# Andreas-Edling/raytracer-rs

Hardware: AMD Instinct MI355X
Metric: Mrays/s (whole node) + ms/frame, 1920x1080x64spp thai2.dae (higher is better)
Workload: dtype f32

## Files before the change

include/mi355rt.h:

```cpp
#ifndef MI355RT_H
#define MI355RT_H

#include <stddef.h>
#include <stdint.h>

#ifdef __cplusplus
extern "C" {
#endif

#define MI355RT_OK            0
#define MI355RT_E_INVALID    -1
#define MI355RT_E_NO_DEVICE  -2
#define MI355RT_E_LOAD       -3
#define MI355RT_E_HIP        -4

#define MI355RT_DEFAULT_TRIANGLES_PER_LEAF 70u
#define MI355RT_DEFAULT_STRIPE_ROWS 4u

#define MI355RT_FLAG_FIX_ROW_INDEX  1u
#define MI355RT_FLAG_COUNT_STEPS    2u
#define MI355RT_FLAG_TIME_KERNELS   4u
#define MI355RT_FLAG_OCTREE_SEMANTICS 8u
#define MI355RT_FLAG_TRUE_CLOSEST_HIT 32u
#define MI355RT_FLAG_GROUP_SHARES_DEVICE 16u
// ... 200 lines not shown
void mi355rt_lens_default(mi355rt_lens* lens);
int  mi355rt_set_lens(mi355rt_handle* h, const mi355rt_lens* lens);
int  mi355rt_get_lens(const mi355rt_handle* h, mi355rt_lens* lens);
int  mi355rt_lens_ray(const float rot16[16], const float orient16[16], const float max_xy[2], uint32_t width, uint32_t height, uint32_t flags,
                      const mi355rt_lens* lens, uint32_t pixel, float xi1, float xi2, float l1, float l2, float ray6[6]);
int  mi355rt_lens_rays(mi355rt_handle* h, uint32_t spp, uint32_t where, float* rays6, size_t nrays);

int mi355rt_get_sample_table(const mi355rt_handle* h, float* out);
int mi355rt_debug_sample(mi355rt_handle* h, uint32_t pixel, uint32_t sampleno, float color3[3], float* node_L, size_t nodes);
int mi355rt_debug_numerics(mi355rt_handle* h, const float* a, const float* b, size_t n, float* quot, float* root, float* pow32);
int mi355rt_debug_slab(mi355rt_handle* h, const float* inv_rays6, const float* cubes6, size_t n, uint8_t* hit, float* tmin);
uint32_t mi355rt_tree_nodes(const mi355rt_handle* h);
int mi355rt_debug_speculation(const mi355rt_handle* h, uint64_t out[2]);
int mi355rt_debug_light_map(const float* tri_verts, uint32_t ntri, const float light[3], double pad, uint32_t res, float* out_dist2, double* nearest);
int mi355rt_debug_reflect_mask(const float* tri_verts, uint32_t ntri, double pad, uint32_t bins, uint64_t work_budget, uint32_t* out_words, double info[8]);

int mi355rt_debug_wide_bvh(const float* tri_verts, uint32_t ntri, uint32_t out[8]);

int mi355rt_accel_stats(const mi355rt_handle* h, uint32_t out[8]);
int mi355rt_reflect_mask_info(const mi355rt_handle* h, double out[4]);
int mi355rt_debug_rays_read(const mi355rt_handle* h, uint64_t* out);
int mi355rt_bvh_build_info(const mi355rt_handle* h, uint32_t out[2]);
int mi355rt_octree_stats(const mi355rt_handle* h, uint32_t out[8]);
uint32_t mi355rt_device_count(const mi355rt_handle* h);
int mi355rt_debug_gather_rate(mi355rt_handle* h, uint32_t table_nodes, uint32_t steps, double out[3]);
int64_t mi355rt_debug_check_guards(mi355rt_handle* h);
uint64_t mi355rt_hbm_allocated_bytes(const mi355rt_handle* h);
int mi355rt_synchronize(mi355rt_handle* h);

#define MI355RT_COMM_ID_BYTES 128
int mi355rt_comm_unique_id(uint8_t* id128);
int mi355rt_comm_available(mi355rt_handle* h);
int mi355rt_comm_init(mi355rt_handle* h, const uint8_t* id128);
int mi355rt_comm_gather_frame(mi355rt_handle* h, uint32_t root, uint32_t* host_out, size_t n);
int mi355rt_comm_destroy(mi355rt_handle* h);
// ... 12 lines not shown
```

raytracer-rs_amd/__init__.py:

```python
import ctypes as C
import os
import sys
import time
import weakref

import numpy as np

DEFAULT_TRIANGLES_PER_LEAF = 70

FLAG_FIX_ROW_INDEX = 1
FLAG_COUNT_STEPS = 2
FLAG_TIME_KERNELS = 4
FLAG_OCTREE_SEMANTICS = 8
FLAG_GROUP_SHARES_DEVICE = 16
FLAG_TRUE_CLOSEST_HIT = 32
FLAG_DEVICE_LBVH = 64
FLAG_DIRECT_FILM = 128

_HERE = os.path.dirname(os.path.abspath(__file__))
LIB_PATH = os.environ.get("MI355RT_LIB") or os.path.join(_HERE, "libmi355rt.so")
_lib = None


class Material(C.Structure):
# ... 170 lines not shown
    ("mi355rt_trace_rays", C.c_int, [_H, C.c_void_p, C.c_void_p, C.c_size_t, C.c_uint32, C.POINTER(RayOutputs)]),
    ("mi355rt_render_rays", C.c_int, [_H, C.c_void_p, C.c_size_t, C.c_uint32, C.c_uint32, C.POINTER(RayCounts)]),
    ("mi355rt_lens_default", None, [C.POINTER(Lens)]),
    ("mi355rt_set_lens", C.c_int, [_H, C.POINTER(Lens)]),
    ("mi355rt_get_lens", C.c_int, [_H, C.POINTER(Lens)]),
    ("mi355rt_lens_ray", C.c_int, [_F, _F, _F, C.c_uint32, C.c_uint32, C.c_uint32, C.POINTER(Lens), C.c_uint32, C.c_float, C.c_float, C.c_float, C.c_float, _F]),
    ("mi355rt_lens_rays", C.c_int, [_H, C.c_uint32, C.c_uint32, C.c_void_p, C.c_size_t]),
    ("mi355rt_get_sample_table", C.c_int, [_H, _F]),
    ("mi355rt_debug_sample", C.c_int, [_H, C.c_uint32, C.c_uint32, _F, _F, C.c_size_t]),
    ("mi355rt_debug_numerics", C.c_int, [_H, _F, _F, C.c_size_t, _F, _F, _F]),
    ("mi355rt_debug_slab", C.c_int, [_H, _F, _F, C.c_size_t, C.POINTER(C.c_uint8), _F]),
    ("mi355rt_tree_nodes", C.c_uint32, [_H]),
    ("mi355rt_debug_speculation", C.c_int, [_H, C.POINTER(C.c_uint64)]),
    ("mi355rt_debug_light_map", C.c_int, [_F, C.c_uint32, _F, C.c_double, C.c_uint32, _F, C.POINTER(C.c_double)]),
    ("mi355rt_debug_reflect_mask", C.c_int, [_F, C.c_uint32, C.c_double, C.c_uint32, C.c_uint64, _U, C.POINTER(C.c_double)]),
    ("mi355rt_reflect_mask_info", C.c_int, [_H, C.POINTER(C.c_double)]),
    ("mi355rt_debug_rays_read", C.c_int, [_H, C.POINTER(C.c_uint64)]),
    ("mi355rt_debug_wide_bvh", C.c_int, [_F, C.c_uint32, _U]),
    ("mi355rt_accel_stats", C.c_int, [_H, _U]),
    ("mi355rt_octree_stats", C.c_int, [_H, _U]),
    ("mi355rt_bvh_build_info", C.c_int, [_H, _U]),
    ("mi355rt_device_count", C.c_uint32, [_H]),
    ("mi355rt_synchronize", C.c_int, [_H]),
    ("mi355rt_comm_unique_id", C.c_int, [C.POINTER(C.c_uint8)]),
    ("mi355rt_comm_available", C.c_int, [_H]),
    ("mi355rt_comm_init", C.c_int, [_H, C.POINTER(C.c_uint8)]),
    ("mi355rt_comm_gather_frame", C.c_int, [_H, C.c_uint32, _U, C.c_size_t]),
    ("mi355rt_comm_destroy", C.c_int, [_H]),
    ("mi355rt_comm_ranks", C.c_uint32, [_H]),
    ("mi355rt_hbm_allocated_bytes", C.c_uint64, [_H]),
# ... 474 lines not shown

    def debug_slab(self, inv_rays6, cubes6):
        r = np.ascontiguousarray(inv_rays6, np.float32).reshape(-1, 6); c = np.ascontiguousarray(cubes6, np.float32).reshape(-1, 6)
        assert r.shape == c.shape
        hit = np.zeros(r.shape[0], np.uint8); tmin = np.zeros(r.shape[0], np.float32)
        self._check(lib().mi355rt_debug_slab(self._h, _fp(r), _fp(c), r.shape[0], hit.ctypes.data_as(C.POINTER(C.c_uint8)), _fp(tmin)))
        return hit.astype(bool), tmin

    def accel_stats(self):
        out = np.zeros(8, np.uint32)
        self._check(lib().mi355rt_accel_stats(self._h, _up(out)))
        return dict(nodes=int(out[0]), leaves=int(out[1]), max_depth=int(out[2]), max_leaf=int(out[3]),
                    node_bytes=int(out[4]), tri_bytes=int(out[5]), bvh_build_ms=int(out[6]) / 1000.0, octree_build_ms=int(out[7]) / 1000.0)

    def reflect_mask_info(self):
        out = (C.c_double * 4)()
        self._check(lib().mi355rt_reflect_mask_info(self._h, out))
        return dict(bins=int(out[0]), build_ms=float(out[1]), clear_share=float(out[2]), bytes=int(out[3]))

    def debug_rays_read(self):
        out = C.c_uint64(0)
        self._check(lib().mi355rt_debug_rays_read(self._h, C.byref(out)))
        return int(out.value)

    def bvh_build_info(self):
        out = np.zeros(2, np.uint32)
        self._check(lib().mi355rt_bvh_build_info(self._h, _up(out)))
        return dict(on_device=bool(out[0]), device_ms=int(out[1]) / 1000.0)

    def octree_stats(self):
        out = np.zeros(8, np.uint32)
        self._check(lib().mi355rt_octree_stats(self._h, _up(out)))
        return dict(nodes=int(out[0]), inner=int(out[1]), leaves=int(out[2]), empty=int(out[3]), depth=int(out[4]), tri_refs=int(out[5]))
# ... 96 lines not shown

def debug_reflect_mask(tri_verts, pad, bins=8, work_budget=0, min_cos=0.0, pad_angle=0.0):
    v = np.ascontiguousarray(tri_verts, np.float32).reshape(-1, 9)
    info = (C.c_double * 8)()
    info[4], info[5] = float(min_cos), float(pad_angle)
    stride = 6 * bins * bins // 32 + 4
    out = np.zeros((v.shape[0], stride), np.uint32)
    code = lib().mi355rt_debug_reflect_mask(_fp(v), v.shape[0], float(pad), int(bins), int(work_budget), _up(out), info)
    if code != 0:
        raise RuntimeError("mi355rt_debug_reflect_mask failed: %d" % code)
    d = dict(stride=int(info[0]), build_ms=float(info[1]), work=int(info[2]), clear_bits=int(info[3]), min_cos=float(info[4]), pad_angle=float(info[5]),
             bary_margin=float(info[6]), built=bool(info[7]))
    return (out if d["built"] else None), d


def debug_wide_bvh(tri_verts):
    v = np.ascontiguousarray(tri_verts, np.float32).reshape(-1, 9)
    out = (C.c_uint32 * 8)()
    code = lib().mi355rt_debug_wide_bvh(_fp(v), v.shape[0], out)
    if code != 0:
        raise RuntimeError("mi355rt_debug_wide_bvh failed: %d" % code)
    keys = ("wide_nodes", "binary_nodes", "stack_need", "binary_depth", "children", "tris_once_wide", "bad_boxes", "tris_once_binary")
    return dict(zip(keys, (int(x) for x in out)))


def comm_unique_id():
    buf = (C.c_uint8 * 128)()
    if lib().mi355rt_comm_unique_id(buf) != 0:
        raise RuntimeError((lib().mi355rt_last_error(None) or b"").decode() or "mi355rt_comm_unique_id failed")
    return bytes(buf)
# ... 29 lines not shown
```

raytracer-rs_amd/csrc/capi.cpp:

```cpp
#include <cmath>
#include <cstdio>
#include <cstring>
#include <exception>
#include <memory>
#include <string>
#include <vector>
#include "display.hpp"
#include "lightmap.hpp"
#include "reflmask.hpp"
#include "../../include/mi355rt.h"
#include "group.hpp"
#include "lens.hpp"
#include "renderer.hpp"

using namespace mi355rt;

namespace mi355rt { bool comm_unique_id(uint8_t* id128, std::string& err); }

struct mi355rt_handle {
    std::unique_ptr<DeviceGroup> g;
    Renderer* r;
    std::string error;
};

// ... 721 lines not shown
    mi355rt::LightMap lm;
    mi355rt::build_light_map(tri_verts, ntri, light, pad, res, lm);
    std::memcpy(out_dist2, lm.dist2.data(), lm.dist2.size() * sizeof(float));
    if (nearest) *nearest = lm.nearest;
    return MI355RT_OK;
}
int mi355rt_debug_reflect_mask(const float* tri_verts, uint32_t ntri, double pad, uint32_t bins, uint64_t work_budget, uint32_t* out_words, double info[8])
{
    if ((ntri && !tri_verts) || !info || !(pad >= 0.0)) return MI355RT_E_INVALID;
    mi355rt::ReflMask m;
    const double min_cos = info[4] > 0.0 ? info[4] : mi355rt::kReflMinCos, pad_angle = info[5] > 0.0 ? info[5] : mi355rt::kReflPadAngle;
    const bool built = ntri != 0 && mi355rt::build_reflect_mask(tri_verts, ntri, pad, bins, work_budget ? work_budget : ~0ull, m, min_cos, pad_angle);
    info[0] = (double)mi355rt::refl_mask_stride(bins); info[1] = m.build_ms; info[2] = (double)m.work; info[3] = (double)m.clear_bits;
    info[4] = min_cos; info[5] = pad_angle; info[6] = (double)mi355rt::kReflBary; info[7] = built ? 1.0 : 0.0;
    if (built && out_words) std::memcpy(out_words, m.words.data(), m.words.size() * sizeof(uint32_t));
    return MI355RT_OK;
}

namespace {
struct WideWalk {
    const mi355rt::Bvh& b; std::vector<uint32_t> seen; uint32_t children = 0, bad_boxes = 0;
    void below(int32_t ref, double mn[3], double mx[3])
    {
        for (int a = 0; a < 3; ++a) { mn[a] = 1e300; mx[a] = -1e300; }
        if (ref < 0) {
            const uint32_t code = ~(uint32_t)ref, first = code >> 3, cnt = (code & 7u) + 1u;
            for (uint32_t t = first; t < first + cnt && t < b.tris.size(); ++t) {
                const mi355rt::BvhTri& r = b.tris[t];
                if (r.prim < seen.size()) ++seen[r.prim];
                for (int v = 0; v < 3; ++v) for (int a = 0; a < 3; ++a) {
// ... 60 lines not shown
    out[6] = (uint32_t)(h->r->build_ms_[0] * 1000.0); out[7] = (uint32_t)(h->r->build_ms_[1] * 1000.0);
    return MI355RT_OK;
}
int mi355rt_bvh_build_info(const mi355rt_handle* h, uint32_t out[2])
{
    if (!h || !out) return MI355RT_E_INVALID;
    out[0] = h->r->bvh_on_device_ ? 1u : 0u; out[1] = (uint32_t)(h->r->lbvh_device_ms_ * 1000.0);
    return MI355RT_OK;
}
int mi355rt_debug_rays_read(const mi355rt_handle* h, uint64_t* out)
{
    if (!h || !out) return MI355RT_E_INVALID;
    *out = h->r->rays_read_;
    return MI355RT_OK;
}
int mi355rt_reflect_mask_info(const mi355rt_handle* h, double out[4])
{
    if (!h || !out) return MI355RT_E_INVALID;
    std::memcpy(out, h->r->reflect_mask_info_, sizeof h->r->reflect_mask_info_);
    return MI355RT_OK;
}
int mi355rt_octree_stats(const mi355rt_handle* h, uint32_t out[8])
{
    if (!h || !out) return MI355RT_E_INVALID;
    std::memcpy(out, h->r->oct_stats_, sizeof h->r->oct_stats_);
    return MI355RT_OK;
}
uint32_t mi355rt_device_count(const mi355rt_handle* h) { return h ? (uint32_t)h->g->size() : 0u; }

int mi355rt_debug_gather_rate(mi355rt_handle* h, uint32_t table_nodes, uint32_t steps, double out[3])
{
// ... 65 lines not shown
```

raytracer-rs_amd/csrc/device_types.hpp:

```cpp
#pragma once
#include <cstdint>
#include <hip/hip_vector_types.h>

namespace mi355rt {

constexpr uint32_t kNumSamples = 65536;
constexpr uint32_t kSampleMax = 65535;
constexpr uint32_t kMaxRecursions = 3;
constexpr uint32_t kMaxLevels = kMaxRecursions + 1;

constexpr uint32_t kRayRecordBytes = 32;
constexpr uint32_t kShards = 64;
constexpr uint32_t kMaxRounds = kMaxRecursions + 2;
constexpr uint32_t kCullRects = 16;
constexpr uint32_t kMaxCursors = 64;
constexpr uint32_t kCtrlWordsPerRound = kMaxCursors * 16384;
constexpr uint32_t kShadeCursorOffset = 128;
constexpr uint32_t kConfirmCursorOffset = 64;
constexpr uint32_t kLiveCountOffset = 192;

struct DMaterial { float r, g, b; uint32_t kind_tex; };
struct DLight { float px, py, pz, cr, cg, cb;
                float tail2;
                float pad; };
// ... 4 lines not shown
    const void* tris;
    const void* normals;
    const DMaterial* materials;
    const DLight* lights;
    const DTexture* textures;
    const float* texels;
    const void* table;
    const void* oct_nodes;
    const uint32_t* oct_leaf_tris;
    const void* prim_tris;
    const int2* oct_info;
    const uint32_t* tri_home;
    const float* light_maps;
    uint32_t light_map_res;
    const uint32_t* refl_mask;
    uint32_t refl_bins, refl_stride;
    int32_t root;
    uint32_t nlights;
    uint32_t ntri;
    uint32_t oct_single_leaf;
    float oct_root[6];
};

constexpr uint32_t kLensPinhole = 0u, kLensThin = 1u, kLensOrtho = 2u;
struct DLens {
    uint32_t model; float radius, focus, width_world;
    float hw, hh, hw2, hh2;
    float axis[3];
    float mx2, my2;
};
// ... 92 lines not shown
```

raytracer-rs_amd/csrc/kernels.hip:

```cpp
#include <hip/hip_runtime.h>
#include <algorithm>
#include <stdint.h>
#include <stdlib.h>
#include <map>
#include <mutex>
#include <utility>
#include "device_math.hpp"
#include "device_types.hpp"
#include "kernels.hpp"
#include "lens.hpp"
#include "reflmask.hpp"
#include "traverse.hpp"

namespace mi355rt {

typedef const uint32_t __attribute__((address_space(4))) * const_u1_ptr;
constexpr int kBlock = 256;
constexpr int kWavesPerBlock = kBlock / 64;
constexpr uint32_t kMiss = 0xFFFFFFFFu;
constexpr int kPrimaryBlocks = 7;
#ifndef MI355RT_WIDE_BLOCKS
#define MI355RT_WIDE_BLOCKS 5
#endif
constexpr int kConfirmBlocks = 5;
// ... 658 lines not shown
    if (ax >= ay && ax >= az) { m = 0u; vm = vx; va = vy; vb = vz; }
    else if (ay >= az) { m = 1u; vm = vy; va = vx; vb = vz; }
    else { m = 2u; vm = vz; va = vx; vb = vy; }
    const float am = fabsf(vm);
    if (!(am > 0.0f) || !(l2 < 3.0e38f)) return false;
    const float fR = (float)R, u = div_rn(va, am), v = div_rn(vb, am);
    const int i = min(max((int)((u * 0.5f + 0.5f) * fR), 0), (int)R - 1), j = min(max((int)((v * 0.5f + 0.5f) * fR), 0), (int)R - 1);
    const uint32_t face = 2u * m + (vm < 0.0f ? 1u : 0u);
    const float bound = sc.light_maps[((size_t)(li * 6u + face) * R + (uint32_t)i) * R + (uint32_t)j];
    return (l2 * 0.98011f < bound) & (l2 * 1.0002e-4f < lt.tail2);
}

__device__ __forceinline__ uint32_t reflection_record(const DScene& sc, const float4 h)
{
    if (sc.refl_mask == nullptr || !((h.y > kReflBary) & (h.z > kReflBary) & (h.y + h.z < 1.0f - kReflBary))) return kMiss;
    return __float_as_uint(h.w) * sc.refl_stride;
}
__device__ __forceinline__ bool reflection_proves_miss(const DScene& sc, uint32_t rec_first, const f3 n, const f3 bo, const f3 bd)
{
    if (rec_first == kMiss) return false;
    const float ax = fabsf(bd.x), ay = fabsf(bd.y), az = fabsf(bd.z);
    uint32_t m; float vm, va, vb;
    if (ax >= ay && ax >= az) { m = 0u; vm = bd.x; va = bd.y; vb = bd.z; }
    else if (ay >= az) { m = 1u; vm = bd.y; va = bd.x; vb = bd.z; }
    else { m = 2u; vm = bd.z; va = bd.x; vb = bd.y; }
    const float am = fabsf(vm);
    if (!(am > 0.0f)) return false;
    const uint32_t B = sc.refl_bins;
    const float fB = (float)B, u = div_rn(va, am), v = div_rn(vb, am);
    const int i = min(max((int)((u * 0.5f + 0.5f) * fB), 0), (int)B - 1), j = min(max((int)((v * 0.5f + 0.5f) * fB), 0), (int)B - 1);
    const uint32_t bit = ((2u * m + (vm < 0.0f ? 1u : 0u)) * B + (uint32_t)i) * B + (uint32_t)j;
    const uint32_t* __restrict__ rec = sc.refl_mask + rec_first;
    if ((rec[bit >> 5] >> (bit & 31u)) & 1u) return false;
    const float4 g = *(const float4*)(rec + (sc.refl_stride - kReflGuardWords));
    return dot3(sub3(bo, mk3(g.x, g.y, g.z)), n) > g.w;
}

template <bool PRIMARY, class List, bool WALK = false, bool RASTER = false, uint32_t RAYS = kFeedCamera>
__device__ __forceinline__ void shade_chunk(const DScene& sc, const DCamera& cam, const DPass& ps, uint32_t level, uint32_t chunk, const List list,
                                            const float4* __restrict__ in_q, uint32_t in_nrad, uint32_t& out_nrad, uint32_t& out_nshadow,
                                            const float4* __restrict__ hits,
                                            float4* __restrict__ out_q, uint2* __restrict__ out_counts,
                                            float* __restrict__ slot_L, uint32_t* __restrict__ sample_slot,
                                            const uint32_t* __restrict__ film_n, DCounters* counters,
                                            unsigned long long& acc_bounce, unsigned long long& acc_shadow, unsigned long long& acc_hits,
                                            float4* lds_hits = nullptr, unsigned long long* acc_tris = nullptr)
{
    const int lane = lane_id();
    {
        uint32_t n_rad = PRIMARY ? min(ps.chunk, ps.nsamples - chunk * ps.chunk) : in_nrad;
// ... 118 lines not shown
                        pcg4d(a0, a1, a2, a3);
                        uint32_t jx0 = __umulhi(a0, 65535u), jx1 = jx0;
                        if (two) {
                            uint32_t b0 = pixel, b1 = sampleno, b2 = 1u + child1, b3 = ps.seed;
                            pcg4d(b0, b1, b2, b3);
                            jx1 = __umulhi(b0, 65535u);
                        }
                        float4 tv0 = table[jx0], tv1 = table[jx1];
                        hemisphere_walk(table, n, jx0, tv0);
                        if (two) hemisphere_walk(table, n, jx1, tv1);
                        bd0 = mk3(tv0.x, tv0.y, tv0.z); bo0 = add3(hp, sscale(0.00001f, bd0));
                        bd1 = mk3(tv1.x, tv1.y, tv1.z); bo1 = add3(hp, sscale(0.00001f, bd1));
                    }
                    bool make0 = active, make1 = active && two;
                    if (sc.refl_mask != nullptr) {
                        if (make0) make0 = !reflection_proves_miss(sc, refl_rec, n, bo0, bd0);
                        if (make1) make1 = !reflection_proves_miss(sc, refl_rec, n, bo1, bd1);
                        bskipped += (uint32_t)__popcll(__ballot(active && !make0)) + (uint32_t)__popcll(__ballot(active && two && !make1));
                    }
                    uint32_t pos[2] = { 0u, 0u };
                    const uint32_t key0 = make0 ? dir_bin(bd0) : kSortBins, key1 = make1 ? dir_bin(bd1) : kSortBins;
                    for (uint32_t b = 0; b < kSortBins; ++b) {
                        const unsigned long long m0 = __ballot(key0 == b), m1 = __ballot(key1 == b);
                        if (key0 == b) pos[0] = out_front + (uint32_t)__popcll(m0 & lanemask_lt());
                        out_front += (uint32_t)__popcll(m0);
                        if (key1 == b) pos[1] = out_front + (uint32_t)__popcll(m1 & lanemask_lt());
                        out_front += (uint32_t)__popcll(m1);
                    }
                    for (uint32_t w = 0; w < (two ? 2u : 1u); ++w) {
                        const f3 bo = w ? bo1 : bo0, bd = w ? bd1 : bd0;
                        const uint32_t child_node = w ? child1 : child0;
                        const uint32_t oi = pos[w];
// ... 1080 lines not shown
```

raytracer-rs_amd/csrc/reflmask.cpp:

```cpp
#include "reflmask.hpp"
#include <algorithm>
#include <atomic>
#include <chrono>
#include <cmath>
#include <cstring>
#include <limits>
#include <thread>

namespace mi355rt {
namespace {

struct V3 { double x, y, z; };
inline V3 sub(V3 a, V3 b) { return { a.x - b.x, a.y - b.y, a.z - b.z }; }
inline V3 add(V3 a, V3 b) { return { a.x + b.x, a.y + b.y, a.z + b.z }; }
inline V3 mul(V3 a, double s) { return { a.x * s, a.y * s, a.z * s }; }
inline double dot(V3 a, V3 b) { return a.x * b.x + a.y * b.y + a.z * b.z; }
inline V3 cross(V3 a, V3 b) { return { a.y * b.z - a.z * b.y, a.z * b.x - a.x * b.z, a.x * b.y - a.y * b.x }; }
inline double len(V3 a) { return std::sqrt(dot(a, a)); }
inline bool unit(V3& a) { const double l = len(a); if (!(l > 0.0) || !std::isfinite(l)) return false; a = mul(a, 1.0 / l); return true; }

const int kAxisA[3] = { 1, 0, 0 }, kAxisB[3] = { 2, 2, 1 };

struct Bin {
    V3 corner[4];
// ... 68 lines not shown
    const std::vector<Bin>& bins;
    const std::vector<Bin>& groups;
    uint32_t B;
    const Tree& tree;
    const float* verts;
    double pad, min_cos, pad_angle, sin_pad;
    uint32_t nbits;
    struct Cap { V3 centre; double cos_rho, sin_rho; };
    std::vector<Cap> bcap, gcap;
    std::vector<uint16_t> clear[24];
    uint32_t nclear = 0;
    V3 normal = { 0, 0, 1 };
    double up_sin;
    std::vector<uint16_t> touched, cand;
    uint64_t work = 0, exacts = 0;

    Walker(const std::vector<Bin>& b, const std::vector<Bin>& g, uint32_t B_, const Tree& t, const float* v, double p, double mc, double pa)
        : bins(b), groups(g), B(B_), tree(t), verts(v), pad(p), min_cos(mc), pad_angle(pa), sin_pad(std::sin(pa)), nbits((uint32_t)b.size()), up_sin(std::sqrt(1.0 - mc * mc))
    {
        for (const Bin& x : b) bcap.push_back(Cap{ x.centre, x.cos_rho, x.sin_rho });
        for (const Bin& x : g) gcap.push_back(Cap{ x.centre, x.cos_rho, x.sin_rho });
    }
    uint32_t group_of(uint32_t b) const { const uint32_t j = b % B, i = (b / B) % B, f = b / (B * B); return f * 4u + (i >= B / 2u ? 2u : 0u) + (j >= B / 2u ? 1u : 0u); }

    static V3 vert(const float* v, int q) { return { v[3 * q], v[3 * q + 1], v[3 * q + 2] }; }

    void cap_touch(V3 d, double cos_half, double sin_half)
    {
        touched.clear();
        {
// ... 78 lines not shown
            cand.assign(touched.begin(), touched.end());
            touched.clear();
            for (uint16_t b : cand) {
                const Bin& bn = bins[b];
                bool separated = false;
                for (int s = 0; s < nsup && !separated; ++s) {
                    bool in = true;
                    for (int k = 0; k < 4; ++k) if (!(dot(sup[s], bn.corner[k]) > sin_pad + 1e-9)) { in = false; break; }
                    separated = in;
                }
                if (!separated) touched.push_back(b);
            }
        }
        cand.assign(touched.begin(), touched.end());
        set_bins(cand, row);
    }

    void triangle(uint32_t t, uint32_t* row, uint32_t stride)
    {
        const uint32_t mask_words = stride - kReflGuardWords;
        for (uint32_t k = 0; k < mask_words; ++k) row[k] = 0xFFFFFFFFu;
        const float* v = verts + 9 * (size_t)t;
        std::memcpy(&row[mask_words], v, 12);
        float hmin = std::numeric_limits<float>::infinity();
        std::memcpy(&row[mask_words + 3], &hmin, 4);
        for (int k = 0; k < 9; ++k) if (!std::isfinite(v[k])) return;
        const V3 p0 = vert(v, 0), p1 = vert(v, 1), p2 = vert(v, 2);
        V3 n = cross(sub(p1, p0), sub(p2, p0));
        const double area2 = len(n);
        const double emax = std::max(len(sub(p1, p0)), std::max(len(sub(p2, p0)), len(sub(p2, p1))));
// ... 58 lines not shown
};

}

bool build_reflect_mask(const float* tri_verts, uint32_t ntri, double pad, uint32_t B, uint64_t work_budget, ReflMask& out, double min_cos, double pad_angle)
{
    out = ReflMask{};
    if (ntri == 0 || B < 4 || B > 16 || (6u * B * B) % 128u != 0u || !(pad >= 0.0) || !(min_cos > 0.0 && min_cos < 1.0) || !(pad_angle >= 0.0 && pad_angle < 0.1)) return false;
    const auto t0 = std::chrono::steady_clock::now();
    const uint32_t stride = refl_mask_stride(B);
    std::vector<Bin> bins, groups; make_bins(B, bins); make_bins(2, groups);
    Tree tree; tree.verts = tri_verts; tree.order.resize(ntri);
    for (uint32_t i = 0; i < ntri; ++i) tree.order[i] = i;
    tree.nodes.reserve((size_t)ntri);
    tree.build(0, ntri);
    std::vector<uint32_t> words((size_t)ntri * stride);
    std::atomic<uint32_t> next{ 0 };
    std::atomic<uint64_t> work{ 0 }, exacts{ 0 };
    std::atomic<bool> over{ false };
    auto worker = [&]() {
        Walker w(bins, groups, B, tree, tri_verts, pad, min_cos, pad_angle);
        for (;;) {
            const uint32_t first = next.fetch_add(64u);
            if (first >= ntri || over.load()) break;
            for (uint32_t t = first; t < std::min(first + 64u, ntri); ++t) w.triangle(t, &words[(size_t)t * stride], stride);
            if (work.fetch_add(w.work) + w.work > work_budget) over.store(true);
            w.work = 0;
            exacts.fetch_add(w.exacts); w.exacts = 0;
        }
    };
    const uint32_t nthreads = std::max(1u, std::min({ 16u, std::thread::hardware_concurrency(), (ntri + 255u) / 256u }));
    std::vector<std::thread> pool;
    for (uint32_t i = 1; i < nthreads; ++i) pool.emplace_back(worker);
    worker();
    for (std::thread& th : pool) th.join();
    out.work = work.load(); out.exact_tests = exacts.load();
    out.build_ms = std::chrono::duration<double, std::milli>(std::chrono::steady_clock::now() - t0).count();
    if (over.load()) return false;
    uint64_t clear_bits = 0;
    for (uint32_t t = 0; t < ntri; ++t) for (uint32_t k = 0; k < stride - kReflGuardWords; ++k) clear_bits += 32u - (uint32_t)__builtin_popcount(words[(size_t)t * stride + k]);
    out.bins = B; out.stride = stride; out.words.swap(words); out.clear_bits = clear_bits;
    return true;
}

}
```

raytracer-rs_amd/csrc/reflmask.hpp:

```cpp
#pragma once
#include <cstdint>
#include <vector>

namespace mi355rt {

constexpr double kReflMinCos = 0.05;
constexpr double kReflPadAngle = 1e-3;
constexpr float kReflBary = 0.02f;
constexpr double kReflHeightUlps = 16.0;
constexpr uint32_t kReflBins = 8;
constexpr uint32_t kReflGuardWords = 4;

struct ReflMask {
    uint32_t bins = 0;
    uint32_t stride = 0;
    std::vector<uint32_t> words;
    double build_ms = 0.0;
    uint64_t work = 0;
    uint64_t exact_tests = 0;
    uint64_t clear_bits = 0;
};

inline uint32_t refl_mask_stride(uint32_t bins) { return 6u * bins * bins / 32u + kReflGuardWords; }

bool build_reflect_mask(const float* tri_verts, uint32_t ntri, double pad, uint32_t bins, uint64_t work_budget, ReflMask& out,
                        double min_cos = kReflMinCos, double pad_angle = kReflPadAngle);

}
```

raytracer-rs_amd/csrc/renderer.cpp:

```cpp
#include "renderer.hpp"
#include "display.hpp"
#include "lightmap.hpp"
#include "reflmask.hpp"
#include <algorithm>
#include <array>
#include <chrono>
#include <cmath>
#include <cstdio>
#include <cstdlib>
#include <cstring>
#include "kernels.hpp"
#include "lens.hpp"
#include "octree.hpp"

namespace mi355rt {

namespace {
void pcg4d(uint32_t v[4])
{
    for (int i = 0; i < 4; ++i) v[i] = v[i] * 1664525u + 1013904223u;
    v[0] += v[1] * v[3]; v[1] += v[2] * v[0]; v[2] += v[0] * v[1]; v[3] += v[1] * v[2];
    for (int i = 0; i < 4; ++i) v[i] ^= v[i] >> 16;
    v[0] += v[1] * v[3]; v[1] += v[2] * v[0]; v[2] += v[0] * v[1]; v[3] += v[1] * v[2];
}
// ... 187 lines not shown
            if (!std::isfinite(l.pos[0]) || !std::isfinite(l.pos[1]) || !std::isfinite(l.pos[2])) { finite = false; break; }
            LightMap lm; build_light_map(scene.tri_verts.data(), ntri, l.pos, pad, res, lm);
            all.insert(all.end(), lm.dist2.begin(), lm.dist2.end());
            const double tail = std::max(lm.nearest - pad, 0.0);
            lights[i].tail2 = std::isfinite(tail) ? (float)std::min(tail * tail * (1.0 - 1e-6), 3.0e38) : 3.0e38f;
            if ((double)lights[i].tail2 > tail * tail) lights[i].tail2 = std::nextafterf(lights[i].tail2, 0.0f);
        }
        if (finite) {
            if (!upload(d_light_maps, all.data(), all.size() * sizeof(float))) return bail();
            light_map_res = res;
        }
        light_map_ms_ = std::chrono::duration<double, std::milli>(std::chrono::steady_clock::now() - t_lm).count();
        if (getenv("MI355RT_DEBUG_CULL")) fprintf(stderr, "[mi355rt] light maps: %zu lights, %u texels per face edge, %.1f ms\n", scene.lights.size(), light_map_res, light_map_ms_);
    }
    if (!upload(d_lights, lights.data(), lights.size() * sizeof(DLight))) return bail();
    uint32_t* d_refl_mask = nullptr; uint32_t refl_bins = 0, refl_stride = 0;
    if (ntri > 0 && cfg.recursions > 0 && !getenv("MI355RT_NO_REFLECT_MASK")) {
        double diag2 = 0.0;
        { float mn[3] = { 3e38f, 3e38f, 3e38f }, mx[3] = { -3e38f, -3e38f, -3e38f };
          for (size_t i = 0; i < scene.tri_verts.size(); ++i) { const int a = (int)(i % 3); mn[a] = std::min(mn[a], scene.tri_verts[i]); mx[a] = std::max(mx[a], scene.tri_verts[i]); }
          for (int a = 0; a < 3; ++a) diag2 += ((double)mx[a] - mn[a]) * ((double)mx[a] - mn[a]); }
        uint64_t budget = 4000000000ull;
        if (const char* e = getenv("MI355RT_REFLECT_MASK_WORK")) budget = std::strtoull(e, nullptr, 10);
        ReflMask rm;
        if (std::isfinite(diag2) && build_reflect_mask(scene.tri_verts.data(), ntri, 2e-4 * std::sqrt(diag2) + 1e-7, kReflBins, budget, rm)) {
            if (!upload(d_refl_mask, rm.words.data(), rm.words.size() * sizeof(uint32_t))) return bail();
            refl_bins = rm.bins; refl_stride = rm.stride;
            reflect_mask_info_[2] = (double)rm.clear_bits / ((double)ntri * 6.0 * rm.bins * rm.bins);
            reflect_mask_info_[3] = (double)(rm.words.size() * sizeof(uint32_t));
        }
        reflect_mask_info_[0] = (double)refl_bins; reflect_mask_info_[1] = rm.build_ms;
        if (getenv("MI355RT_DEBUG_CULL")) fprintf(stderr, "[mi355rt] reflection masks: %u bins per face edge, %.1f ms, %llu work units, %.3f of the bits clear\n", refl_bins, rm.build_ms, (unsigned long long)rm.work, reflect_mask_info_[2]);
    }
    std::vector<DTexture> tex(std::max<size_t>(scene.textures.size(), 1));
    std::vector<float> texels;
    for (size_t i = 0; i < scene.textures.size(); ++i) {
        const TextureData& t = scene.textures[i];
        if (t.rgb.size() != (size_t)t.width * t.height * 3 || t.rgb.empty()) { err = "texture size mismatch"; code = MI355RT_E_INVALID; return false; }
        tex[i] = DTexture{ t.width, t.height, texels.size() / 3 };
        texels.insert(texels.end(), t.rgb.begin(), t.rgb.end());
    }
    if (!upload(d_tex, tex.data(), tex.size() * sizeof(DTexture))) return bail();
    if (!upload(d_texels, texels.data(), texels.size() * sizeof(float))) return bail();
    dscene_.nodes = d_nodes; dscene_.tris = d_tris; dscene_.normals = d_normals; dscene_.materials = d_mats;
    dscene_.lights = d_lights; dscene_.textures = d_tex; dscene_.texels = d_texels; dscene_.table = d_table;
    dscene_.root = bvh.root; dscene_.nlights = nlights_; dscene_.ntri = ntri;
    dscene_.light_maps = d_light_maps; dscene_.light_map_res = light_map_res;
    dscene_.refl_mask = d_refl_mask; dscene_.refl_bins = refl_bins; dscene_.refl_stride = refl_stride;
    dscene_.oct_nodes = nullptr; dscene_.oct_leaf_tris = nullptr; dscene_.prim_tris = nullptr; dscene_.oct_info = nullptr; dscene_.tri_home = nullptr; dscene_.oct_single_leaf = 0u;
    std::memset(dscene_.oct_root, 0, sizeof dscene_.oct_root);
    mode_ = (cfg.flags & MI355RT_FLAG_OCTREE_SEMANTICS) ? kModeOctreeWalk : (cfg.flags & MI355RT_FLAG_TRUE_CLOSEST_HIT) ? kModeTrueClosest : kModeConfirm;
    if (mode_ != kModeTrueClosest) {
        Octree oct;
        const auto t_oct = std::chrono::steady_clock::now();
        build_octree(scene.tri_verts.data(), ntri, cfg.triangles_per_leaf, oct);
        build_ms_[1] = std::chrono::duration<double, std::milli>(std::chrono::steady_clock::now() - t_oct).count();
        oct_stats_[0] = (uint32_t)oct.nodes.size(); oct_stats_[1] = oct.inner; oct_stats_[2] = oct.leaves;
        oct_stats_[3] = oct.empty_leaves; oct_stats_[4] = oct.max_depth; oct_stats_[5] = (uint32_t)oct.leaf_tris.size();
        std::vector<BvhTri> prim_tris(std::max(ntri, 1u));
        std::memset(prim_tris.data(), 0, prim_tris.size() * sizeof(BvhTri));
        for (uint32_t t = 0; t < ntri; ++t) {
            const float* v = &scene.tri_verts[9 * (size_t)t];
            for (int a = 0; a < 3; ++a) { prim_tris[t].v0[a] = v[a]; prim_tris[t].e1[a] = v[3 + a] - v[a]; prim_tris[t].e2[a] = v[6 + a] - v[a]; }
// ... 1389 lines not shown
```

raytracer-rs_amd/csrc/renderer.hpp:

```cpp
#pragma once
#include <hip/hip_runtime_api.h>
#include <array>
#include <memory>
#include <string>
#include <vector>
#include "../../include/mi355rt.h"
#include "bvh.hpp"
#include "camera.hpp"
#include "device_buffer.hpp"
#include "device_types.hpp"
#include "scene.hpp"

namespace mi355rt {

class Renderer {
public:
    static std::unique_ptr<Renderer> create(const SceneData& scene, const mi355rt_config& cfg, std::string& err, int& code);
    ~Renderer();

    uint32_t trace_frame_additive();
    bool render(uint32_t spp, bool wait = true);
    bool render_adaptive(const mi355rt_adaptive_config& ac, mi355rt_adaptive_stats& st);
    bool adaptive_tile_mask(const mi355rt_adaptive_config& ac, uint8_t* out, uint32_t& active);
    uint32_t tiles_x() const { return (cfg.width + kAdaptiveTile - 1) / kAdaptiveTile; }
// ... 60 lines not shown
    std::vector<std::array<float, 6>> cull_boxes_;
    size_t hbm_bytes_ = 0;
    DeviceBuffer<uint32_t> d_cull_mask_;
    std::vector<float> mask_key_;
    float mask_dom_[4] = { 0, 0, 0, 0 };
    bool mask_valid_ = false;
    DeviceBuffer<uint2> d_tile_ofs_, d_tile_entries_;
    std::vector<float> bins_key_;
    uint32_t bins_layout_[3] = { 0, 0, 0 };
    bool bins_valid_ = false;
    double bins_ms_ = 0.0; size_t bins_entries_ = 0;
    uint32_t oct_stats_[8] = { 0 };
    double build_ms_[2] = { 0.0, 0.0 };
    double light_map_ms_ = 0.0;
    uint64_t rays_read_ = 0;
    double reflect_mask_info_[4] = { 0.0, 0.0, 0.0, 0.0 };
    bool bvh_on_device_ = false;
    bool wide_ = false;
    uint32_t traversal_rows() const { return (wide_ ? bvh.stack_need4 : bvh.max_depth) + 1u; }
    double lbvh_device_ms_ = 0.0;
    enum Mode { kModeConfirm = 0, kModeOctreeWalk = 1, kModeTrueClosest = 2 };
    Mode mode_ = kModeConfirm;

private:
    Renderer() = default;
    bool init(const SceneData& scene, std::string& err, int& code);
    bool bind();
    bool fail(hipError_t e, const char* what);
    struct Slice {
        hipStream_t stream = nullptr;
        hipEvent_t done = nullptr;
// ... 115 lines not shown
```

Baseline: 20600.

## Prove reflection-ray misses near the surface with per-triangle self-clearance records

```diff
diff --git a/include/mi355rt.h b/include/mi355rt.h
--- a/include/mi355rt.h
+++ b/include/mi355rt.h
@@ -238,11 +238,12 @@
 int mi355rt_debug_speculation(const mi355rt_handle* h, uint64_t out[2]);
 int mi355rt_debug_light_map(const float* tri_verts, uint32_t ntri, const float light[3], double pad, uint32_t res, float* out_dist2, double* nearest);
 int mi355rt_debug_reflect_mask(const float* tri_verts, uint32_t ntri, double pad, uint32_t bins, uint64_t work_budget, uint32_t* out_words, double info[8]);
+int mi355rt_debug_reflect_self(const float* tri_verts, uint32_t ntri, double pad, uint32_t bins, uint64_t work_budget, uint32_t* out_words, double info[8]);
 
 int mi355rt_debug_wide_bvh(const float* tri_verts, uint32_t ntri, uint32_t out[8]);
 
 int mi355rt_accel_stats(const mi355rt_handle* h, uint32_t out[8]);
-int mi355rt_reflect_mask_info(const mi355rt_handle* h, double out[4]);
+int mi355rt_reflect_mask_info(const mi355rt_handle* h, double out[5]);
 int mi355rt_debug_rays_read(const mi355rt_handle* h, uint64_t* out);
 int mi355rt_bvh_build_info(const mi355rt_handle* h, uint32_t out[2]);
 int mi355rt_octree_stats(const mi355rt_handle* h, uint32_t out[8]);
diff --git a/raytracer-rs_amd/__init__.py b/raytracer-rs_amd/__init__.py
--- a/raytracer-rs_amd/__init__.py
+++ b/raytracer-rs_amd/__init__.py
@@ -208,6 +208,7 @@
     ("mi355rt_debug_speculation", C.c_int, [_H, C.POINTER(C.c_uint64)]),
     ("mi355rt_debug_light_map", C.c_int, [_F, C.c_uint32, _F, C.c_double, C.c_uint32, _F, C.POINTER(C.c_double)]),
     ("mi355rt_debug_reflect_mask", C.c_int, [_F, C.c_uint32, C.c_double, C.c_uint32, C.c_uint64, _U, C.POINTER(C.c_double)]),
+    ("mi355rt_debug_reflect_self", C.c_int, [_F, C.c_uint32, C.c_double, C.c_uint32, C.c_uint64, _U, C.POINTER(C.c_double)]),
     ("mi355rt_reflect_mask_info", C.c_int, [_H, C.POINTER(C.c_double)]),
     ("mi355rt_debug_rays_read", C.c_int, [_H, C.POINTER(C.c_uint64)]),
     ("mi355rt_debug_wide_bvh", C.c_int, [_F, C.c_uint32, _U]),
@@ -712,9 +713,9 @@
                     node_bytes=int(out[4]), tri_bytes=int(out[5]), bvh_build_ms=int(out[6]) / 1000.0, octree_build_ms=int(out[7]) / 1000.0)
 
     def reflect_mask_info(self):
-        out = (C.c_double * 4)()
+        out = (C.c_double * 5)()
         self._check(lib().mi355rt_reflect_mask_info(self._h, out))
-        return dict(bins=int(out[0]), build_ms=float(out[1]), clear_share=float(out[2]), bytes=int(out[3]))
+        return dict(bins=int(out[0]), build_ms=float(out[1]), clear_share=float(out[2]), bytes=int(out[3]), self_allowed=int(out[4]))
 
     def debug_rays_read(self):
         out = C.c_uint64(0)
@@ -841,6 +842,19 @@
     return (out if d["built"] else None), d
 
 
+def debug_reflect_self(tri_verts, pad, bins=8, work_budget=0, min_cos=0.0, pad_angle=0.0):
+    v = np.ascontiguousarray(tri_verts, np.float32).reshape(-1, 9)
+    info = (C.c_double * 8)()
+    info[4], info[5] = float(min_cos), float(pad_angle)
+    out = np.zeros((v.shape[0], 8), np.uint32)
+    code = lib().mi355rt_debug_reflect_self(_fp(v), v.shape[0], float(pad), int(bins), int(work_budget), _up(out), info)
+    if code != 0:
+        raise RuntimeError("mi355rt_debug_reflect_self failed: %d" % code)
+    d = dict(words=int(info[0]), allowed=int(info[1]), floor_ulps=float(info[2]), prism_depth=float(info[3]), min_cos=float(info[4]), pad_angle=float(info[5]),
+             work=int(info[6]), built=bool(info[7]))
+    return (out if d["built"] else None), d
+
+
 def debug_wide_bvh(tri_verts):
     v = np.ascontiguousarray(tri_verts, np.float32).reshape(-1, 9)
     out = (C.c_uint32 * 8)()
diff --git a/raytracer-rs_amd/csrc/capi.cpp b/raytracer-rs_amd/csrc/capi.cpp
--- a/raytracer-rs_amd/csrc/capi.cpp
+++ b/raytracer-rs_amd/csrc/capi.cpp
@@ -759,6 +759,17 @@
     info[0] = (double)mi355rt::refl_mask_stride(bins); info[1] = m.build_ms; info[2] = (double)m.work; info[3] = (double)m.clear_bits;
     info[4] = min_cos; info[5] = pad_angle; info[6] = (double)mi355rt::kReflBary; info[7] = built ? 1.0 : 0.0;
     if (built && out_words) std::memcpy(out_words, m.words.data(), m.words.size() * sizeof(uint32_t));
+    return MI355RT_OK;
+}
+int mi355rt_debug_reflect_self(const float* tri_verts, uint32_t ntri, double pad, uint32_t bins, uint64_t work_budget, uint32_t* out_words, double info[8])
+{
+    if ((ntri && !tri_verts) || !info || !(pad >= 0.0)) return MI355RT_E_INVALID;
+    mi355rt::ReflMask m;
+    const double min_cos = info[4] > 0.0 ? info[4] : mi355rt::kReflMinCos, pad_angle = info[5] > 0.0 ? info[5] : mi355rt::kReflPadAngle;
+    const bool built = ntri != 0 && mi355rt::build_reflect_mask(tri_verts, ntri, pad, bins, work_budget ? work_budget : ~0ull, m, min_cos, pad_angle);
+    info[0] = (double)mi355rt::kReflSelfWords; info[1] = (double)m.self_allowed; info[2] = mi355rt::kReflFloorUlps; info[3] = mi355rt::kReflPrismDepth;
+    info[4] = min_cos; info[5] = pad_angle; info[6] = (double)m.work; info[7] = built ? 1.0 : 0.0;
+    if (built && out_words) std::memcpy(out_words, m.self.data(), m.self.size() * sizeof(uint32_t));
     return MI355RT_OK;
 }
 
@@ -849,7 +860,7 @@
     *out = h->r->rays_read_;
     return MI355RT_OK;
 }
-int mi355rt_reflect_mask_info(const mi355rt_handle* h, double out[4])
+int mi355rt_reflect_mask_info(const mi355rt_handle* h, double out[5])
 {
     if (!h || !out) return MI355RT_E_INVALID;
     std::memcpy(out, h->r->reflect_mask_info_, sizeof h->r->reflect_mask_info_);
diff --git a/raytracer-rs_amd/csrc/device_types.hpp b/raytracer-rs_amd/csrc/device_types.hpp
--- a/raytracer-rs_amd/csrc/device_types.hpp
+++ b/raytracer-rs_amd/csrc/device_types.hpp
@@ -42,6 +42,7 @@
     const float* light_maps;
     uint32_t light_map_res;
     const uint32_t* refl_mask;
+    const float4* refl_self;
     uint32_t refl_bins, refl_stride;
     int32_t root;
     uint32_t nlights;
diff --git a/raytracer-rs_amd/csrc/kernels.hip b/raytracer-rs_amd/csrc/kernels.hip
--- a/raytracer-rs_amd/csrc/kernels.hip
+++ b/raytracer-rs_amd/csrc/kernels.hip
@@ -696,26 +696,42 @@
 __device__ __forceinline__ uint32_t reflection_record(const DScene& sc, const float4 h)
 {
     if (sc.refl_mask == nullptr || !((h.y > kReflBary) & (h.z > kReflBary) & (h.y + h.z < 1.0f - kReflBary))) return kMiss;
-    return __float_as_uint(h.w) * sc.refl_stride;
-}
-__device__ __forceinline__ bool reflection_proves_miss(const DScene& sc, uint32_t rec_first, const f3 n, const f3 bo, const f3 bd)
-{
-    if (rec_first == kMiss) return false;
+    return __float_as_uint(h.w);
+}
+constexpr uint32_t kReflTrace = 0u, kReflProven = 1u, kReflAsk = 2u;
+__device__ __forceinline__ uint32_t reflection_verdict(const DScene& sc, uint32_t prim, const f3 n, const f3 bo, const f3 bd, float4& g, float& hgt)
+{
+    if (prim == kMiss) return kReflTrace;
     const float ax = fabsf(bd.x), ay = fabsf(bd.y), az = fabsf(bd.z);
     uint32_t m; float vm, va, vb;
     if (ax >= ay && ax >= az) { m = 0u; vm = bd.x; va = bd.y; vb = bd.z; }
     else if (ay >= az) { m = 1u; vm = bd.y; va = bd.x; vb = bd.z; }
     else { m = 2u; vm = bd.z; va = bd.x; vb = bd.y; }
     const float am = fabsf(vm);
-    if (!(am > 0.0f)) return false;
+    if (!(am > 0.0f)) return kReflTrace;
     const uint32_t B = sc.refl_bins;
     const float fB = (float)B, u = div_rn(va, am), v = div_rn(vb, am);
     const int i = min(max((int)((u * 0.5f + 0.5f) * fB), 0), (int)B - 1), j = min(max((int)((v * 0.5f + 0.5f) * fB), 0), (int)B - 1);
     const uint32_t bit = ((2u * m + (vm < 0.0f ? 1u : 0u)) * B + (uint32_t)i) * B + (uint32_t)j;
-    const uint32_t* __restrict__ rec = sc.refl_mask + rec_first;
-    if ((rec[bit >> 5] >> (bit & 31u)) & 1u) return false;
-    const float4 g = *(const float4*)(rec + (sc.refl_stride - kReflGuardWords));
-    return dot3(sub3(bo, mk3(g.x, g.y, g.z)), n) > g.w;
+    const uint32_t* __restrict__ rec = sc.refl_mask + prim * sc.refl_stride;
+    if ((rec[bit >> 5] >> (bit & 31u)) & 1u) return kReflTrace;
+    g = *(const float4*)(rec + (sc.refl_stride - kReflGuardWords));
+    const float height = dot3(sub3(bo, mk3(g.x, g.y, g.z)), n);
+    if (height > g.w) return kReflProven;
+    hgt = height;
+    return sc.refl_self != nullptr ? kReflAsk : kReflTrace;
+}
+__device__ __forceinline__ bool reflection_self_accepts(const f3 o, const f3 d, const f3 v0, const f3 v0v1, const f3 v0v2)
+{
+    const f3 pvec = cross3(d, v0v2);
+    const float det = dot3(v0v1, pvec);
+    const float inv_det = div_rn(1.0f, det);
+    const f3 tvec = sub3(o, v0);
+    const float u = dot3(tvec, pvec) * inv_det;
+    const f3 qvec = cross3(tvec, v0v1);
+    const float v = dot3(d, qvec) * inv_det;
+    const float t = dot3(v0v2, qvec) * inv_det;
+    return !(fabsf(det) < 1.1920929e-7f) & !((u < 0.0f) | (u > 1.0f)) & !((v < 0.0f) | (u + v > 1.0f)) & !(t < 0.0f);
 }
 
 template <bool PRIMARY, class List, bool WALK = false, bool RASTER = false, uint32_t RAYS = kFeedCamera>
@@ -864,8 +880,18 @@
                     }
                     bool make0 = active, make1 = active && two;
                     if (sc.refl_mask != nullptr) {
-                        if (make0) make0 = !reflection_proves_miss(sc, refl_rec, n, bo0, bd0);
-                        if (make1) make1 = !reflection_proves_miss(sc, refl_rec, n, bo1, bd1);
+                        float4 g = make_float4(0, 0, 0, 0); float hgt0 = 0.0f, hgt1 = 0.0f;
+                        uint32_t verdict0 = make0 ? reflection_verdict(sc, refl_rec, n, bo0, bd0, g, hgt0) : kReflTrace;
+                        uint32_t verdict1 = make1 ? reflection_verdict(sc, refl_rec, n, bo1, bd1, g, hgt1) : kReflTrace;
+                        if (__ballot((verdict0 == kReflAsk) | (verdict1 == kReflAsk)) != 0ull) {
+                            float4 s0 = make_float4(0, 0, 0, 0), s1 = s0;
+                            if ((verdict0 == kReflAsk) | (verdict1 == kReflAsk)) { const float4* __restrict__ sr = sc.refl_self + 2u * (size_t)refl_rec; s0 = sr[0]; s1 = sr[1]; }
+                            const bool allowed = (__float_as_uint(s1.w) & kReflSelfAllowed) != 0u;
+                            const f3 sv0 = mk3(g.x, g.y, g.z), te1 = mk3(s0.x, s0.y, s0.z), te2 = mk3(s1.x, s1.y, s1.z);
+                            if (verdict0 == kReflAsk) verdict0 = (allowed && hgt0 >= s0.w && !reflection_self_accepts(bo0, bd0, sv0, te1, te2)) ? kReflProven : kReflTrace;
+                            if (verdict1 == kReflAsk) verdict1 = (allowed && hgt1 >= s0.w && !reflection_self_accepts(bo1, bd1, sv0, te1, te2)) ? kReflProven : kReflTrace;
+                        }
+                        make0 = make0 && verdict0 != kReflProven; make1 = make1 && verdict1 != kReflProven;
                         bskipped += (uint32_t)__popcll(__ballot(active && !make0)) + (uint32_t)__popcll(__ballot(active && two && !make1));
                     }
                     uint32_t pos[2] = { 0u, 0u };
diff --git a/raytracer-rs_amd/csrc/reflmask.cpp b/raytracer-rs_amd/csrc/reflmask.cpp
--- a/raytracer-rs_amd/csrc/reflmask.cpp
+++ b/raytracer-rs_amd/csrc/reflmask.cpp
@@ -106,6 +106,7 @@
     double up_sin;
     std::vector<uint16_t> touched, cand;
     uint64_t work = 0, exacts = 0;
+    bool all_finite = true;
 
     Walker(const std::vector<Bin>& b, const std::vector<Bin>& g, uint32_t B_, const Tree& t, const float* v, double p, double mc, double pa)
         : bins(b), groups(g), B(B_), tree(t), verts(v), pad(p), min_cos(mc), pad_angle(pa), sin_pad(std::sin(pa)), nbits((uint32_t)b.size()), up_sin(std::sqrt(1.0 - mc * mc))
@@ -214,6 +215,80 @@
         }
         cand.assign(touched.begin(), touched.end());
         set_bins(cand, row);
+    }
+
+    static bool clip_leaves_something(const float* u9, const V3* a, const double* c, int nplanes)
+    {
+        V3 poly[16], next[16]; int np = 3;
+        for (int q = 0; q < 3; ++q) poly[q] = vert(u9, q);
+        for (int k = 0; k < nplanes && np > 0; ++k) {
+            int nn = 0;
+            for (int i = 0; i < np; ++i) {
+                const V3 p = poly[i], q = poly[(i + 1) % np];
+                const double dp = dot(a[k], p) - c[k], dq = dot(a[k], q) - c[k];
+                if (dp >= 0.0) next[nn++] = p;
+                if ((dp >= 0.0) != (dq >= 0.0)) { const double s = dp / (dp - dq); next[nn++] = add(p, mul(sub(q, p), s)); }
+            }
+            np = nn;
+            for (int i = 0; i < np; ++i) poly[i] = next[i];
+        }
+        return np > 0;
+    }
+
+    void self_record(uint32_t t, const uint32_t* row, uint32_t stride, uint32_t* rec)
+    {
+        const float* v = verts + 9 * (size_t)t;
+        const float e[8] = { v[3] - v[0], v[4] - v[1], v[5] - v[2], 0.0f, v[6] - v[0], v[7] - v[1], v[8] - v[2], 0.0f };
+        std::memcpy(rec, e, sizeof e);
+        float hmin; std::memcpy(&hmin, &row[stride - 1u], 4);
+        if (!std::isfinite(hmin)) return;
+        const V3 p0 = vert(v, 0), p1 = vert(v, 1), p2 = vert(v, 2);
+        V3 n = cross(sub(p1, p0), sub(p2, p0));
+        const double area2 = len(n);
+        const double emax = std::max(len(sub(p1, p0)), std::max(len(sub(p2, p0)), len(sub(p2, p1))));
+        if (!(emax > 0.0) || !unit(n)) return;
+        const double hgt = area2 / emax;
+        double amax = 0.0;
+        for (int k = 0; k < 9; ++k) amax = std::max(amax, std::fabs((double)v[k]));
+        const double bm = 0.5 * (double)kReflBary;
+        const float floor32 = -(float)(kReflFloorUlps * std::ldexp(amax, -23));
+        const double fl = -(double)floor32;
+        if (!(fl > 0.0) || !(fl / min_cos < 0.25 * bm * hgt)) return;
+        std::memcpy(&rec[3], &floor32, 4);
+        if (!all_finite) return;
+        const V3 tp[3] = { add(mul(p0, 1.0 - 2.0 * bm), mul(add(p1, p2), bm)), add(mul(p1, 1.0 - 2.0 * bm), mul(add(p0, p2), bm)), add(mul(p2, 1.0 - 2.0 * bm), mul(add(p0, p1), bm)) };
+        const double depth = kReflPrismDepth * fl, eh = 0.01 * fl, es = 1e-9 * emax;
+        V3 a[5]; double c[5];
+        a[0] = mul(n, -1.0); c[0] = -dot(n, p0) - eh;
+        a[1] = n; c[1] = dot(n, p0) - depth - eh;
+        for (int i = 0; i < 3; ++i) {
+            V3 m = cross(n, sub(tp[(i + 1) % 3], tp[i]));
+            if (!unit(m)) return;
+            if (dot(m, sub(tp[(i + 2) % 3], tp[i])) < 0.0) m = mul(m, -1.0);
+            a[2 + i] = m; c[2 + i] = dot(m, tp[i]) - es;
+        }
+        V3 lo = { 1e300, 1e300, 1e300 }, hi = { -1e300, -1e300, -1e300 };
+        for (int i = 0; i < 3; ++i) for (int s = 0; s < 2; ++s) {
+            const V3 p = s ? sub(tp[i], mul(n, depth)) : tp[i];
+            lo = { std::min(lo.x, p.x), std::min(lo.y, p.y), std::min(lo.z, p.z) }; hi = { std::max(hi.x, p.x), std::max(hi.y, p.y), std::max(hi.z, p.z) };
+        }
+        const double ex = 2.0 * (eh + es);
+        const V3 bc = mul(add(lo, hi), 0.5), bh = add(mul(sub(hi, lo), 0.5), V3{ ex, ex, ex });
+        int32_t stack[128]; int sp = 0;
+        stack[sp++] = 0;
+        while (sp > 0) {
+            const Node& nd = tree.nodes[(size_t)stack[--sp]];
+            ++work;
+            if (std::fabs(nd.c.x - bc.x) > nd.h.x + bh.x || std::fabs(nd.c.y - bc.y) > nd.h.y + bh.y || std::fabs(nd.c.z - bc.z) > nd.h.z + bh.z) continue;
+            if (nd.left < 0) {
+                for (uint32_t k = 0; k < nd.count; ++k) {
+                    const uint32_t u = tree.order[nd.first + k];
+                    if (u != t && clip_leaves_something(verts + 9 * (size_t)u, a, c, 5)) return;
+                }
+            } else if (sp + 2 <= 128) { stack[sp++] = nd.left; stack[sp++] = nd.right; }
+            else return;
+        }
+        rec[7] = kReflSelfAllowed;
     }
 
     void triangle(uint32_t t, uint32_t* row, uint32_t stride)
@@ -302,16 +377,22 @@
     for (uint32_t i = 0; i < ntri; ++i) tree.order[i] = i;
     tree.nodes.reserve((size_t)ntri);
     tree.build(0, ntri);
-    std::vector<uint32_t> words((size_t)ntri * stride);
+    std::vector<uint32_t> words((size_t)ntri * stride), self((size_t)ntri * kReflSelfWords);
+    bool all_finite = true;
+    for (size_t i = 0; i < (size_t)ntri * 9u; ++i) all_finite = all_finite && std::isfinite(tri_verts[i]);
     std::atomic<uint32_t> next{ 0 };
     std::atomic<uint64_t> work{ 0 }, exacts{ 0 };
     std::atomic<bool> over{ false };
     auto worker = [&]() {
         Walker w(bins, groups, B, tree, tri_verts, pad, min_cos, pad_angle);
+        w.all_finite = all_finite;
         for (;;) {
             const uint32_t first = next.fetch_add(64u);
             if (first >= ntri || over.load()) break;
-            for (uint32_t t = first; t < std::min(first + 64u, ntri); ++t) w.triangle(t, &words[(size_t)t * stride], stride);
+            for (uint32_t t = first; t < std::min(first + 64u, ntri); ++t) {
+                w.triangle(t, &words[(size_t)t * stride], stride);
+                w.self_record(t, &words[(size_t)t * stride], stride, &self[(size_t)t * kReflSelfWords]);
+            }
             if (work.fetch_add(w.work) + w.work > work_budget) over.store(true);
             w.work = 0;
             exacts.fetch_add(w.exacts); w.exacts = 0;
@@ -327,7 +408,9 @@
     if (over.load()) return false;
     uint64_t clear_bits = 0;
     for (uint32_t t = 0; t < ntri; ++t) for (uint32_t k = 0; k < stride - kReflGuardWords; ++k) clear_bits += 32u - (uint32_t)__builtin_popcount(words[(size_t)t * stride + k]);
-    out.bins = B; out.stride = stride; out.words.swap(words); out.clear_bits = clear_bits;
+    uint32_t allowed = 0;
+    for (uint32_t t = 0; t < ntri; ++t) allowed += self[(size_t)t * kReflSelfWords + 7u] & kReflSelfAllowed;
+    out.bins = B; out.stride = stride; out.words.swap(words); out.clear_bits = clear_bits; out.self.swap(self); out.self_allowed = allowed;
     return true;
 }
 
diff --git a/raytracer-rs_amd/csrc/reflmask.hpp b/raytracer-rs_amd/csrc/reflmask.hpp
--- a/raytracer-rs_amd/csrc/reflmask.hpp
+++ b/raytracer-rs_amd/csrc/reflmask.hpp
@@ -10,6 +10,10 @@
 constexpr double kReflHeightUlps = 16.0;
 constexpr uint32_t kReflBins = 8;
 constexpr uint32_t kReflGuardWords = 4;
+constexpr double kReflFloorUlps = 8.0;
+constexpr double kReflPrismDepth = 2.0;
+constexpr uint32_t kReflSelfWords = 8;
+constexpr uint32_t kReflSelfAllowed = 1u;
 
 struct ReflMask {
     uint32_t bins = 0;
@@ -19,6 +23,8 @@
     uint64_t work = 0;
     uint64_t exact_tests = 0;
     uint64_t clear_bits = 0;
+    std::vector<uint32_t> self;
+    uint32_t self_allowed = 0;
 };
 
 inline uint32_t refl_mask_stride(uint32_t bins) { return 6u * bins * bins / 32u + kReflGuardWords; }
diff --git a/raytracer-rs_amd/csrc/renderer.cpp b/raytracer-rs_amd/csrc/renderer.cpp
--- a/raytracer-rs_amd/csrc/renderer.cpp
+++ b/raytracer-rs_amd/csrc/renderer.cpp
@@ -225,7 +225,7 @@
         if (getenv("MI355RT_DEBUG_CULL")) fprintf(stderr, "[mi355rt] light maps: %zu lights, %u texels per face edge, %.1f ms\n", scene.lights.size(), light_map_res, light_map_ms_);
     }
     if (!upload(d_lights, lights.data(), lights.size() * sizeof(DLight))) return bail();
-    uint32_t* d_refl_mask = nullptr; uint32_t refl_bins = 0, refl_stride = 0;
+    uint32_t* d_refl_mask = nullptr; uint32_t* d_refl_self = nullptr; uint32_t refl_bins = 0, refl_stride = 0;
     if (ntri > 0 && cfg.recursions > 0 && !getenv("MI355RT_NO_REFLECT_MASK")) {
         double diag2 = 0.0;
         { float mn[3] = { 3e38f, 3e38f, 3e38f }, mx[3] = { -3e38f, -3e38f, -3e38f };
@@ -239,6 +239,11 @@
             refl_bins = rm.bins; refl_stride = rm.stride;
             reflect_mask_info_[2] = (double)rm.clear_bits / ((double)ntri * 6.0 * rm.bins * rm.bins);
             reflect_mask_info_[3] = (double)(rm.words.size() * sizeof(uint32_t));
+            if (!getenv("MI355RT_NO_REFLECT_SELF")) {
+                if (!upload(d_refl_self, rm.self.data(), rm.self.size() * sizeof(uint32_t))) return bail();
+                reflect_mask_info_[3] += (double)(rm.self.size() * sizeof(uint32_t));
+                reflect_mask_info_[4] = (double)rm.self_allowed;
+            }
         }
         reflect_mask_info_[0] = (double)refl_bins; reflect_mask_info_[1] = rm.build_ms;
         if (getenv("MI355RT_DEBUG_CULL")) fprintf(stderr, "[mi355rt] reflection masks: %u bins per face edge, %.1f ms, %llu work units, %.3f of the bits clear\n", refl_bins, rm.build_ms, (unsigned long long)rm.work, reflect_mask_info_[2]);
@@ -257,7 +262,7 @@
     dscene_.lights = d_lights; dscene_.textures = d_tex; dscene_.texels = d_texels; dscene_.table = d_table;
     dscene_.root = bvh.root; dscene_.nlights = nlights_; dscene_.ntri = ntri;
     dscene_.light_maps = d_light_maps; dscene_.light_map_res = light_map_res;
-    dscene_.refl_mask = d_refl_mask; dscene_.refl_bins = refl_bins; dscene_.refl_stride = refl_stride;
+    dscene_.refl_mask = d_refl_mask; dscene_.refl_self = (const float4*)d_refl_self; dscene_.refl_bins = refl_bins; dscene_.refl_stride = refl_stride;
     dscene_.oct_nodes = nullptr; dscene_.oct_leaf_tris = nullptr; dscene_.prim_tris = nullptr; dscene_.oct_info = nullptr; dscene_.tri_home = nullptr; dscene_.oct_single_leaf = 0u;
     std::memset(dscene_.oct_root, 0, sizeof dscene_.oct_root);
     mode_ = (cfg.flags & MI355RT_FLAG_OCTREE_SEMANTICS) ? kModeOctreeWalk : (cfg.flags & MI355RT_FLAG_TRUE_CLOSEST_HIT) ? kModeTrueClosest : kModeConfirm;
diff --git a/raytracer-rs_amd/csrc/renderer.hpp b/raytracer-rs_amd/csrc/renderer.hpp
--- a/raytracer-rs_amd/csrc/renderer.hpp
+++ b/raytracer-rs_amd/csrc/renderer.hpp
@@ -98,7 +98,7 @@
     double build_ms_[2] = { 0.0, 0.0 };
     double light_map_ms_ = 0.0;
     uint64_t rays_read_ = 0;
-    double reflect_mask_info_[4] = { 0.0, 0.0, 0.0, 0.0 };
+    double reflect_mask_info_[5] = { 0.0, 0.0, 0.0, 0.0, 0.0 };
     bool bvh_on_device_ = false;
     bool wide_ = false;
     uint32_t traversal_rows() const { return (wide_ ? bvh.stack_need4 : bvh.max_depth) + 1u; }
```

New measurement: 20770 (median of 6 runs). No clear change (+0.8%).
